# microsoft/tf-gnn-samples

Hardware: AMD Instinct MI355X
Metric: edges/sec (whole node), RGCN PPI h=256 training, distinct batches (the reference's epoch-loop definition) (higher is better)
Workload: dtype f32; 1 GPU; C2: RGCN on synthetic PPI-shaped batches (~16 graphs, ~1.88 M edges, ~32 k nodes each), 3 edge types [fwd,self,bkwd], h=256, 3 layers, sum aggregation, 1/in-de…; graphs_per_rank=64, max_nodes_in_batch=35964, input_pipeline=ResidentDataset, parallelism=dp1-by-graph

## Files before the change

tf_gnn_samples_amd/csrc/plan_resident.hip:

```cpp
#include "common.h"

using namespace relgnn;

namespace {

__device__ __forceinline__ int upper_slot(const int64_t* __restrict__ table, int n, int64_t x) {
  int lo = 0, hi = n;
  while (hi - lo > 1) {
    const int mid = (lo + hi) >> 1;
    if (table[mid] <= x) lo = mid; else hi = mid;
  }
  return lo;
}

struct BatchTables {
  const int64_t* ids;
  const int64_t* node_off_b;
  const int64_t* msg_off_b;
  const int64_t* edge_off_b;
  const int64_t* type_off_b;
  const int64_t* node_off_d;
  const int64_t* msg_off_d;
  const int64_t* edge_off_d;
  const int64_t* type_off_d;
  int32_t K, L;
  int64_t G;
};

__device__ __forceinline__ int32_t translate_message(const BatchTables& t, int32_t m_d, int l, int k, int64_t g) {
  const int64_t e = (int64_t)m_d - t.type_off_d[l] - t.edge_off_d[(int64_t)l * (t.G + 1) + g];
  return (int32_t)(t.type_off_b[l] + t.edge_off_b[(int64_t)l * (t.K + 1) + k] + e);
}

template <bool FULL>
__global__ __launch_bounds__(256) void assemble_by_target_kernel(
    BatchTables t, int64_t M, const int32_t* __restrict__ perm_d, const int32_t* __restrict__ col_d,
    int32_t* __restrict__ perm_b, int32_t* __restrict__ col_b, int32_t* __restrict__ inv_b,
    const float* __restrict__ w_t_d, int32_t* __restrict__ src_b, float* __restrict__ w_t_b) {
  __shared__ int first_slot;
  for (int64_t base = (int64_t)blockIdx.x * 1024; base < M; base += (int64_t)gridDim.x * 1024) {
    if (threadIdx.x == 0) first_slot = upper_slot(t.msg_off_b, t.K, base);
    __syncthreads();
    int k = first_slot;
    int64_t g = t.ids[k], slot_end = t.msg_off_b[k + 1];
    int64_t msg_delta = t.msg_off_d[g] - t.msg_off_b[k], node_delta = t.node_off_b[k] - t.node_off_d[g];
#pragma unroll
    for (int e = 0; e < 4; ++e) {
      const int64_t p = base + threadIdx.x + 256 * e;
      if (p >= M) break;
      if (p >= slot_end) {
        do { ++k; } while (p >= t.msg_off_b[k + 1]);
        g = t.ids[k]; slot_end = t.msg_off_b[k + 1];
        msg_delta = t.msg_off_d[g] - t.msg_off_b[k]; node_delta = t.node_off_b[k] - t.node_off_d[g];
      }
      const int64_t pd = p + msg_delta;
      const uint32_t c = (uint32_t)col_d[pd];
      const uint32_t cn = c / (uint32_t)t.L;
      const int64_t src = (int64_t)cn + node_delta;
      if (src_b) src_b[p] = (int32_t)src;
      if (w_t_b) w_t_b[p] = w_t_d[pd];
      if constexpr (FULL) {
        const int l = (int)(c - cn * (uint32_t)t.L);
        col_b[p] = (int32_t)(src * t.L + l);
        const int32_t mb = translate_message(t, perm_d[pd], l, k, g);
        perm_b[p] = mb;
        inv_b[mb] = (int32_t)p;
      }
    }
    __syncthreads();
  }
}

template <bool FULL>
__global__ __launch_bounds__(256) void assemble_by_source_kernel(
    BatchTables t, int64_t M, const int32_t* __restrict__ perm_d, const int32_t* __restrict__ frow_d,
    const int32_t* __restrict__ pos_d, int32_t* __restrict__ perm_b, int32_t* __restrict__ frow_b,
    int32_t* __restrict__ tgt_b, int32_t* __restrict__ pos_b, const float* __restrict__ w_s_d, float* __restrict__ w_s_b) {
  __shared__ int first_slot;
  for (int64_t base = (int64_t)blockIdx.x * 1024; base < M; base += (int64_t)gridDim.x * 1024) {
    if (threadIdx.x == 0) first_slot = upper_slot(t.msg_off_b, t.K, base);
    __syncthreads();
    int k = first_slot;
    int64_t g = t.ids[k], slot_end = t.msg_off_b[k + 1];
    int64_t msg_delta = t.msg_off_d[g] - t.msg_off_b[k], node_delta = t.node_off_b[k] - t.node_off_d[g];
#pragma unroll
    for (int e = 0; e < 4; ++e) {
      const int64_t q = base + threadIdx.x + 256 * e;
      if (q >= M) break;
      if (q >= slot_end) {
        do { ++k; } while (q >= t.msg_off_b[k + 1]);
        g = t.ids[k]; slot_end = t.msg_off_b[k + 1];
        msg_delta = t.msg_off_d[g] - t.msg_off_b[k]; node_delta = t.node_off_b[k] - t.node_off_d[g];
      }
      const int64_t qd = q + msg_delta;
      const uint32_t f = (uint32_t)frow_d[qd];
      const uint32_t fn = f / (uint32_t)t.L;
      const int64_t tgt = (int64_t)fn + node_delta;
      tgt_b[q] = (int32_t)tgt;
      if (w_s_b) w_s_b[q] = w_s_d[qd];
      if constexpr (FULL) {
        const int l = (int)(f - fn * (uint32_t)t.L);
        frow_b[q] = (int32_t)(tgt * t.L + l);
        perm_b[q] = translate_message(t, perm_d[qd], l, k, g);
        pos_b[q] = (int32_t)((int64_t)pos_d[qd] - msg_delta);
      }
    }
    __syncthreads();
  }
}

__global__ __launch_bounds__(256) void assemble_rowptr_kernel(
    BatchTables t, int64_t num_buckets, int64_t M, const int32_t* __restrict__ rowptr_t_d,
    const int32_t* __restrict__ rowptr_s_d, int32_t* __restrict__ rowptr_t_b, int32_t* __restrict__ rowptr_s_b) {
  for (int64_t b = blockIdx.x * (int64_t)blockDim.x + threadIdx.x; b <= num_buckets; b += (int64_t)gridDim.x * blockDim.x) {
    if (b == num_buckets) {
      rowptr_t_b[b] = (int32_t)M;
      rowptr_s_b[b] = (int32_t)M;
      continue;
    }
    const int64_t v = b / t.L;
    const int l = (int)(b - v * t.L);
    const int k = upper_slot(t.node_off_b, t.K, v);
    const int64_t g = t.ids[k];
    const int64_t bd = (v - t.node_off_b[k] + t.node_off_d[g]) * t.L + l;
    const int64_t shift = t.msg_off_b[k] - t.msg_off_d[g];
    rowptr_t_b[b] = (int32_t)((int64_t)rowptr_t_d[bd] + shift);
    rowptr_s_b[b] = (int32_t)((int64_t)rowptr_s_d[bd] + shift);
  }
}


__global__ __launch_bounds__(256) void gather_node_rows_kernel(BatchTables t, int64_t V, int32_t cols,
                                                               const uint32_t* __restrict__ src, uint32_t* __restrict__ dst) {
  __shared__ int first_slot;
  const int64_t total = V * cols;
  for (int64_t base = (int64_t)blockIdx.x * 1024; base < total; base += (int64_t)gridDim.x * 1024) {
    if (threadIdx.x == 0) {
      int lo = 0, hi = t.K;
      while (hi - lo > 1) {
        const int mid = (lo + hi) >> 1;
        if (t.node_off_b[mid] * cols <= base) lo = mid; else hi = mid;
      }
      first_slot = lo;
    }
    __syncthreads();
    int k = first_slot;
    int64_t slot_end = t.node_off_b[k + 1] * cols;
    int64_t delta = (t.node_off_d[t.ids[k]] - t.node_off_b[k]) * cols;
#pragma unroll
    for (int e = 0; e < 4; ++e) {
      const int64_t i = base + threadIdx.x + 256 * e;
      if (i < total) {
        if (i >= slot_end) {
          do { ++k; } while (i >= t.node_off_b[k + 1] * cols);
          slot_end = t.node_off_b[k + 1] * cols;
          delta = (t.node_off_d[t.ids[k]] - t.node_off_b[k]) * cols;
        }
        dst[i] = src[delta + i];
      }
    }
    __syncthreads();
  }
}

__global__ __launch_bounds__(256) void gather_degree_kernel(BatchTables t, int64_t V, int64_t N, const float* __restrict__ deg_d,
                                                            float* __restrict__ deg_b, int32_t* __restrict__ node_to_graph) {
  for (int64_t v = blockIdx.x * (int64_t)blockDim.x + threadIdx.x; v < V; v += (int64_t)gridDim.x * blockDim.x) {
    const int k = upper_slot(t.node_off_b, t.K, v);
    const int64_t vd = v - t.node_off_b[k] + t.node_off_d[t.ids[k]];
    for (int l = 0; l < t.L; ++l) deg_b[(int64_t)l * V + v] = deg_d[(int64_t)l * N + vd];
    node_to_graph[v] = k;
  }
}

__global__ __launch_bounds__(256) void gather_adjacency_kernel(BatchTables t, int64_t M, const int2* __restrict__ adj_d,
                                                               int2* __restrict__ adj_b) {
  for (int64_t p = blockIdx.x * (int64_t)blockDim.x + threadIdx.x; p < M; p += (int64_t)gridDim.x * blockDim.x) {
    const int l = upper_slot(t.type_off_b, t.L, p);
    const int64_t e = p - t.type_off_b[l];
    const int64_t* eob = t.edge_off_b + (int64_t)l * (t.K + 1);
    const int k = upper_slot(eob, t.K, e);
    const int64_t g = t.ids[k];
    const int64_t pd = t.type_off_d[l] + t.edge_off_d[(int64_t)l * (t.G + 1) + g] + (e - eob[k]);
    int2 a = adj_d[pd];
    const int off = (int)t.node_off_b[k];
    a.x += off; a.y += off;
    adj_b[p] = a;
  }
}

}

extern "C" {

int relgnn_batch_gather(const int64_t* ids, int32_t num_batch_graphs, int32_t num_edge_types, int64_t num_dataset_graphs,
                        const int64_t* node_off_b, const int64_t* edge_off_b, const int64_t* type_off_b,
                        const int64_t* node_off_d, const int64_t* edge_off_d, const int64_t* type_off_d, int64_t num_nodes,
                        int64_t num_messages, int64_t num_dataset_nodes, int32_t n_payloads, const void* const* h_payload_d,
                        const int32_t* h_payload_cols, void* const* h_payload_b, const float* deg_d, float* deg_b,
                        const int32_t* adj_d, int32_t* adj_b, int32_t* node_to_graph, void* stream) {
  if (num_batch_graphs < 0 || num_edge_types <= 0 || num_dataset_graphs < 0 || num_nodes < 0 || num_messages < 0 ||
      n_payloads < 0 || num_dataset_nodes < 0)
    return RELGNN_EINVAL;
  if (num_batch_graphs == 0 || num_nodes == 0) return RELGNN_OK;
  if (!ids || !node_off_b || !edge_off_b || !type_off_b || !node_off_d || !edge_off_d || !type_off_d) return RELGNN_EINVAL;
  if (n_payloads > 0 && (!h_payload_d || !h_payload_cols || !h_payload_b)) return RELGNN_EINVAL;
  hipStream_t st = as_stream(stream);
  BatchTables t{ids, node_off_b, nullptr, edge_off_b, type_off_b, node_off_d, nullptr, edge_off_d, type_off_d,
                num_batch_graphs, num_edge_types, num_dataset_graphs};
  for (int p = 0; p < n_payloads; ++p) {
    if (h_payload_cols[p] <= 0) continue;
    if (!h_payload_d[p] || !h_payload_b[p]) return RELGNN_EINVAL;
    gather_node_rows_kernel<<<flat_grid((num_nodes * h_payload_cols[p] + 3) / 4, 256), 256, 0, st>>>(
        t, num_nodes, h_payload_cols[p], (const uint32_t*)h_payload_d[p], (uint32_t*)h_payload_b[p]);
  }
  if (deg_b || node_to_graph) {
    if (!deg_d || !deg_b || !node_to_graph) return RELGNN_EINVAL;
    gather_degree_kernel<<<flat_grid(num_nodes, 256), 256, 0, st>>>(t, num_nodes, num_dataset_nodes, deg_d, deg_b, node_to_graph);
  }
  if (num_messages > 0 && adj_b) {
    if (!adj_d) return RELGNN_EINVAL;
    gather_adjacency_kernel<<<flat_grid(num_messages, 256), 256, 0, st>>>(t, num_messages, (const int2*)adj_d, (int2*)adj_b);
  }
  return launch_status();
}

int relgnn_plan_assemble(const int64_t* ids, int32_t num_batch_graphs, int32_t num_edge_types, int64_t num_dataset_graphs,
                         const int64_t* node_off_b, const int64_t* msg_off_b, const int64_t* edge_off_b,
                         const int64_t* type_off_b, const int64_t* node_off_d, const int64_t* msg_off_d,
                         const int64_t* edge_off_d, const int64_t* type_off_d, int64_t num_nodes, int64_t num_messages,
                         const int32_t* rowptr_t_d, const int32_t* perm_t_d, const int32_t* col_t_d,
                         const int32_t* rowptr_s_d, const int32_t* perm_s_d, const int32_t* frow_s_d,
                         const int32_t* pos_t_of_s_d, int32_t* rowptr_t, int32_t* perm_t, int32_t* col_t,
                         int32_t* inv_perm_t, int32_t* rowptr_s, int32_t* perm_s, int32_t* frow_s, int32_t* tgt_s,
                         int32_t* pos_t_of_s, const float* w_t_d, const float* w_s_d, int32_t* src_t, float* w_t, float* w_s,
                         void* stream) {
  if (num_batch_graphs < 0 || num_edge_types <= 0 || num_dataset_graphs < 0 || num_nodes < 0 || num_messages < 0)
    return RELGNN_EINVAL;
  const int64_t buckets = num_nodes * num_edge_types;
  if (buckets >= INT32_MAX || num_messages >= INT32_MAX) return RELGNN_EUNSUPPORTED;
  if (!rowptr_t || !rowptr_s) return RELGNN_EINVAL;
  hipStream_t st = as_stream(stream);
  if (num_batch_graphs == 0 || num_nodes == 0) {
    if (hipMemsetAsync(rowptr_t, 0, (size_t)(buckets + 1) * 4, st) != hipSuccess) return RELGNN_EHIP;
    if (hipMemsetAsync(rowptr_s, 0, (size_t)(buckets + 1) * 4, st) != hipSuccess) return RELGNN_EHIP;
    return RELGNN_OK;
  }
  if (!ids || !node_off_b || !msg_off_b || !edge_off_b || !type_off_b || !node_off_d || !msg_off_d || !edge_off_d ||
      !type_off_d || !rowptr_t_d || !rowptr_s_d)
    return RELGNN_EINVAL;
  BatchTables t{ids, node_off_b, msg_off_b, edge_off_b, type_off_b, node_off_d, msg_off_d, edge_off_d, type_off_d,
                num_batch_graphs, num_edge_types, num_dataset_graphs};
  assemble_rowptr_kernel<<<flat_grid(buckets + 1, 256), 256, 0, st>>>(t, buckets, num_messages, rowptr_t_d, rowptr_s_d,
                                                                      rowptr_t, rowptr_s);
  if (num_messages > 0) {
    const bool full = perm_t || col_t || inv_perm_t || perm_s || frow_s || pos_t_of_s;
    if (full && (!perm_t || !col_t || !inv_perm_t || !perm_s || !frow_s || !pos_t_of_s || !perm_t_d || !perm_s_d || !pos_t_of_s_d))
      return RELGNN_EINVAL;
    if (!col_t_d || !frow_s_d || !tgt_s) return RELGNN_EINVAL;
    if (!full && !src_t) return RELGNN_EINVAL;
    if ((w_t && !w_t_d) || (w_s && !w_s_d)) return RELGNN_EINVAL;
    const dim3 grid = flat_grid((num_messages + 3) / 4, 256);
    if (full) {
      assemble_by_target_kernel<true><<<grid, 256, 0, st>>>(t, num_messages, perm_t_d, col_t_d, perm_t, col_t, inv_perm_t,
                                                            w_t_d, src_t, w_t);
      assemble_by_source_kernel<true><<<grid, 256, 0, st>>>(t, num_messages, perm_s_d, frow_s_d, pos_t_of_s_d, perm_s, frow_s,
                                                            tgt_s, pos_t_of_s, w_s_d, w_s);
    } else {
      assemble_by_target_kernel<false><<<grid, 256, 0, st>>>(t, num_messages, nullptr, col_t_d, nullptr, nullptr, nullptr,
                                                             w_t_d, src_t, w_t);
      assemble_by_source_kernel<false><<<grid, 256, 0, st>>>(t, num_messages, nullptr, frow_s_d, nullptr, nullptr, nullptr,
                                                             tgt_s, nullptr, w_s_d, w_s);
    }
  }
  return launch_status();
}

}
```

tf_gnn_samples_amd/csrc/train_utils.hip:

```cpp
#include "common.h"
#include "adam_element.h"
#include "norm_tree.h"
#include "../../include/relgnn_subgraph_norm.h"
#include <type_traits>

using namespace relgnn;

namespace {

struct MtArgs {
  float* p[RELGNN_MT_MAX];
  const float* g[RELGNN_MT_MAX];
  float* m[RELGNN_MT_MAX];
  float* v[RELGNN_MT_MAX];
  long long n[RELGNN_MT_MAX];
};

struct NormArgs {
  const float* g[RELGNN_MT_MAX];
  long long n[RELGNN_MT_MAX];
};

__device__ __forceinline__ double block_sum_1024(double x, double* red) {
#pragma unroll
  for (int off = 32; off >= 1; off >>= 1) x += __shfl_xor(x, off);
  const int wave = threadIdx.x >> 6, lane = threadIdx.x & 63;
  if (lane == 0) red[wave] = x;
  __syncthreads();
  double t = 0.0;
  if (threadIdx.x == 0)
    for (int i = 0; i < (int)(blockDim.x >> 6); ++i) t += red[i];
  __syncthreads();
  return t;
}

__global__ __launch_bounds__(kNormBlock) void mt_l2norm_partial_kernel(NormArgs a, double* __restrict__ partial) {
  __shared__ double red[4];
  const int t = blockIdx.y;
  const float* g = a.g[t];
  const long long n = a.n[t];
  double acc = 0.0;
  for (long long i = (long long)blockIdx.x * blockDim.x + threadIdx.x; i < n; i += (long long)gridDim.x * blockDim.x) {
    const double x = g[i];
    acc += x * x;
  }
  const double sum = norm_block_partial(acc, red);
  if (threadIdx.x == 0) partial[(long long)t * kNormChunks + blockIdx.x] = sum;
}

__global__ __launch_bounds__(64) void mt_l2norm_final_kernel(const double* __restrict__ partial, float* __restrict__ norms) {
  const int t = blockIdx.x;
  const float norm = norm_of_partials(partial + (long long)t * kNormChunks);
  if (threadIdx.x == 0) norms[t] = norm;
}

__global__ void adam_step_size_kernel(float* __restrict__ state, float lr, float b1, float b2) {
  const float t = state[0] + 1.f;
  state[0] = t;
  state[1] = lr * sqrtf(1.f - powf(b2, t)) / (1.f - powf(b1, t));
}

__global__ __launch_bounds__(256) void mt_adam_clip_kernel(MtArgs a, const float* __restrict__ norms, float clip,
                                                           float lr_t, const float* __restrict__ d_lr_t, float b1, float b2,
                                                           float eps) {
  if (d_lr_t) lr_t = d_lr_t[0];
  const int t = blockIdx.y;
  const long long n = a.n[t];
  const long long chunk = 4096;
  const long long beg = (long long)blockIdx.x * chunk;
  if (beg >= n) return;
  const long long end = min(n, beg + chunk);
  float scale = 1.f;
  if (clip > 0.f) {
    const float nrm = norms[t];
    scale = clip / fmaxf(nrm, clip);
  }
  float* p = a.p[t];
  const float* g = a.g[t];
  float* m = a.m[t];
  float* v = a.v[t];
  for (long long i = beg + threadIdx.x; i < end; i += blockDim.x) {
    float pi = p[i], mi = m[i], vi = v[i];
    adam_element(pi, g[i] * scale, mi, vi, lr_t, b1, b2, eps);
    m[i] = mi;
    v[i] = vi;
    p[i] = pi;
  }
}

struct SgdArgs {
  float* p[RELGNN_MT_MAX];
  const float* g[RELGNN_MT_MAX];
  long long n[RELGNN_MT_MAX];
};

__device__ __forceinline__ void rmsprop_element(float& p, float g, float& ms, float& mom, float scale, float lr,
                                                float one_minus_decay, float momentum, float eps) {
#pragma clang fp contract(off)
  const float gi = g * scale;
  const float d = gi * gi - ms;
  ms = ms + d * one_minus_decay;
  const float num = lr * gi;
  mom = mom * momentum + num / sqrtf(ms + eps);
  p = p - mom;
}

__device__ __forceinline__ void sgd_element(float& p, float g, float scale, float lr) {
#pragma clang fp contract(off)
  const float gi = g * scale;
  p = p - lr * gi;
}

__device__ __forceinline__ float clip_scale(const float* __restrict__ norms, int t, float clip) {
  return clip > 0.f ? clip / fmaxf(norms[t], clip) : 1.f;
}

__device__ __forceinline__ bool aligned16(const void* a, const void* b, const void* c = nullptr, const void* d = nullptr) {
  return ((reinterpret_cast<uintptr_t>(a) | reinterpret_cast<uintptr_t>(b) | reinterpret_cast<uintptr_t>(c) |
           reinterpret_cast<uintptr_t>(d)) & 15) == 0;
}

__global__ __launch_bounds__(256) void mt_rmsprop_clip_kernel(MtArgs a, const float* __restrict__ norms, float clip, float lr,
                                                              float decay, float momentum, float eps) {
  const int t = blockIdx.y;
  const long long n = a.n[t];
  const long long beg = (long long)blockIdx.x * 4096;
  if (beg >= n) return;
  const int len = (int)min(n - beg, 4096LL);
  const float scale = clip_scale(norms, t, clip);
  const float omd = 1.f - decay;
  float* p = a.p[t] + beg;
  const float* g = a.g[t] + beg;
  float* ms = a.m[t] + beg;
  float* mom = a.v[t] + beg;
  const int n4 = aligned16(p, g, ms, mom) ? len / 4 : 0;
  for (int i = threadIdx.x; i < n4; i += blockDim.x) {
    float4 pv = reinterpret_cast<float4*>(p)[i], sv = reinterpret_cast<float4*>(ms)[i], mv = reinterpret_cast<float4*>(mom)[i];
    const float4 gv = reinterpret_cast<const float4*>(g)[i];
    rmsprop_element(pv.x, gv.x, sv.x, mv.x, scale, lr, omd, momentum, eps);
    rmsprop_element(pv.y, gv.y, sv.y, mv.y, scale, lr, omd, momentum, eps);
    rmsprop_element(pv.z, gv.z, sv.z, mv.z, scale, lr, omd, momentum, eps);
    rmsprop_element(pv.w, gv.w, sv.w, mv.w, scale, lr, omd, momentum, eps);
    reinterpret_cast<float4*>(ms)[i] = sv;
    reinterpret_cast<float4*>(mom)[i] = mv;
    reinterpret_cast<float4*>(p)[i] = pv;
  }
  for (int i = 4 * n4 + threadIdx.x; i < len; i += blockDim.x) {
    float pi = p[i], si = ms[i], mi = mom[i];
    rmsprop_element(pi, g[i], si, mi, scale, lr, omd, momentum, eps);
    ms[i] = si;
    mom[i] = mi;
    p[i] = pi;
  }
}

__global__ __launch_bounds__(256) void mt_sgd_clip_kernel(SgdArgs a, const float* __restrict__ norms, float clip, float lr) {
  const int t = blockIdx.y;
  const long long n = a.n[t];
  const long long beg = (long long)blockIdx.x * 4096;
  if (beg >= n) return;
  const int len = (int)min(n - beg, 4096LL);
  const float scale = clip_scale(norms, t, clip);
  float* p = a.p[t] + beg;
  const float* g = a.g[t] + beg;
  const int n4 = aligned16(p, g) ? len / 4 : 0;
  for (int i = threadIdx.x; i < n4; i += blockDim.x) {
    float4 pv = reinterpret_cast<float4*>(p)[i];
    const float4 gv = reinterpret_cast<const float4*>(g)[i];
    sgd_element(pv.x, gv.x, scale, lr);
    sgd_element(pv.y, gv.y, scale, lr);
    sgd_element(pv.z, gv.z, scale, lr);
    sgd_element(pv.w, gv.w, scale, lr);
    reinterpret_cast<float4*>(p)[i] = pv;
  }
  for (int i = 4 * n4 + threadIdx.x; i < len; i += blockDim.x) {
    float pi = p[i];
    sgd_element(pi, g[i], scale, lr);
    p[i] = pi;
  }
}

struct CeAcc {
  double loss;
  int tp, fp, fn;
};

__device__ __forceinline__ void ce_element(float x, float z, CeAcc& a) {
  const float e = expf(-fabsf(x));
  a.loss += (double)(fmaxf(x, 0.f) - x * z + log1pf(e));
  const bool pred = sigmoid_label(x, e);
  const int zi = (int)z;
  a.tp += (pred && zi != 0) ? 1 : 0;
  a.fp += (pred && zi != 1) ? 1 : 0;
  a.fn += (!pred && zi != 0) ? 1 : 0;
}

__global__ __launch_bounds__(1024) void sigmoid_ce_stats_kernel(const float* __restrict__ logits,
                                                                const float* __restrict__ labels, long long n,
                                                                double* __restrict__ partial) {
  __shared__ double red[16];
  CeAcc a = {0.0, 0, 0, 0};
  const long long tid = (long long)blockIdx.x * blockDim.x + threadIdx.x, nth = (long long)gridDim.x * blockDim.x;
  const bool vec = ((reinterpret_cast<uintptr_t>(logits) | reinterpret_cast<uintptr_t>(labels)) & 15) == 0;
  const long long n4 = vec ? n / 4 : 0;
  const float4* x4 = reinterpret_cast<const float4*>(logits);
  const float4* z4 = reinterpret_cast<const float4*>(labels);
  for (long long i = tid; i < n4; i += nth) {
    const float4 x = x4[i], z = z4[i];
    ce_element(x.x, z.x, a); ce_element(x.y, z.y, a); ce_element(x.z, z.z, a); ce_element(x.w, z.w, a);
  }
  for (long long i = 4 * n4 + tid; i < n; i += nth) ce_element(logits[i], labels[i], a);
  double s;
  s = block_sum_1024(a.loss, red);       if (threadIdx.x == 0) partial[blockIdx.x * 4 + 0] = s;
  s = block_sum_1024((double)a.tp, red); if (threadIdx.x == 0) partial[blockIdx.x * 4 + 1] = s;
  s = block_sum_1024((double)a.fp, red); if (threadIdx.x == 0) partial[blockIdx.x * 4 + 2] = s;
  s = block_sum_1024((double)a.fn, red); if (threadIdx.x == 0) partial[blockIdx.x * 4 + 3] = s;
}

__global__ __launch_bounds__(256) void sigmoid_ce_stats_final_kernel(const double* __restrict__ partial, int nblk,
                                                                     float mean_scale, float* __restrict__ stats) {
  __shared__ double red[4][4];
  __shared__ double tot[4];
  const int b = threadIdx.x;
  double v[4];
#pragma unroll
  for (int k = 0; k < 4; ++k) v[k] = b < nblk ? partial[b * 4 + k] : 0.0;
#pragma unroll
  for (int k = 0; k < 4; ++k) {
#pragma unroll
    for (int off = 32; off >= 1; off >>= 1) v[k] += __shfl_xor(v[k], off);
  }
  const int wave = b >> 6, lane = b & 63;
  if (lane == 0) {
#pragma unroll
    for (int k = 0; k < 4; ++k) red[wave][k] = v[k];
  }
  __syncthreads();
  if (b < 4) {
    const double s = (red[0][b] + red[1][b]) + (red[2][b] + red[3][b]);
    stats[b] = (float)s;
    tot[b] = s;
  }
  __syncthreads();
  if (b == 0) {
    const double precision = tot[1] / (tot[1] + tot[2]);
    const double recall = tot[1] / (tot[1] + tot[3]);
    stats[4] = (float)((2.0 * precision * recall) / (precision + recall));
    stats[5] = (float)tot[0] * mean_scale;
  }
}

__global__ __launch_bounds__(256) void sigmoid_ce_bwd_kernel(const float* __restrict__ logits,
                                                             const float* __restrict__ labels, long long n,
                                                             const float* __restrict__ g_mean, float mean_scale,
                                                             const float* __restrict__ g_total, float* __restrict__ gl) {
  float gs = 0.f;
  if (g_mean) gs = g_mean[0] * mean_scale;
  if (g_total) gs = g_mean ? gs + g_total[0] : g_total[0];
  for (long long i = (long long)blockIdx.x * blockDim.x + threadIdx.x; i < n; i += (long long)gridDim.x * blockDim.x) {
    const float x = logits[i];
    gl[i] = gs * (1.f / (1.f + expf(-x)) - labels[i]);
  }
}

__global__ __launch_bounds__(256) void sigmoid_ce_bwd_padded_kernel(const float* __restrict__ logits,
                                                                    const float* __restrict__ labels, long long rows, int cols,
                                                                    int ldg, const float* __restrict__ g_mean, float mean_scale,
                                                                    const float* __restrict__ g_total, float* __restrict__ gl) {
  float gs = 0.f;
  if (g_mean) gs = g_mean[0] * mean_scale;
  if (g_total) gs = g_mean ? gs + g_total[0] : g_total[0];
  const long long n = rows * ldg;
// ... 149 lines not shown
                                                                      const int* __restrict__ labels, const float* __restrict__ mask,
                                                                      const float* __restrict__ weights, float denominator,
                                                                      long long rows, int cols, const float* __restrict__ g_loss,
                                                                      const float* __restrict__ g_total, float* __restrict__ gl,
                                                                      long long ldg) {
  constexpr int kRowsPerBlock = 256 / W;
  const int j = threadIdx.x % W, g = threadIdx.x / W;
  float gs = 0.f;
  if (g_loss) gs = g_loss[0] / denominator;
  if (g_total) gs = g_loss ? gs + g_total[0] : g_total[0];
  for (long long base = (long long)blockIdx.x * kRowsPerBlock; base < rows; base += (long long)gridDim.x * kRowsPerBlock) {
    const long long r = base + g;
    const bool valid = r < rows;
    const float* row = logits + (valid ? r : 0) * ld;
    const RowLse a = row_lse<W>(row, valid ? cols : 0, j);
    if (!valid) continue;
    const float mk = mask[r];
    const int label = labels[r];
    const float scale = (mk * weights[r]) * gs, inv = 1.f / (1.f + a.t);
    float* out = gl + r * ldg;
    for (int c = j; c < (int)ldg; c += W) {
      float v = 0.f;
      if (c < cols && mk != 0.f) v = scale * (expf(row[c] - a.m) * inv - (c == label ? 1.f : 0.f));
      out[c] = v;
    }
  }
}

constexpr int kSoftmaxBlocks = 256;

static inline int softmax_grid(long long rows, int w) {
  const long long per_block = 256 / w;
  long long g = (rows + per_block - 1) / per_block;
  return (int)(g < 1 ? 1 : (g > kSoftmaxBlocks ? kSoftmaxBlocks : g));
}

template <bool kWeighted>
int softmax_ce_stats_launch(const float* logits, int64_t ld, const int32_t* labels, const float* mask, const float* weights,
                            float denominator, int64_t rows, int32_t cols, float* stats, void* workspace, size_t workspace_bytes,
                            void* stream) {
  if (rows < 0 || cols < 1 || ld < cols || !stats || (kWeighted && (denominator == 0.f || denominator != denominator)))
    return RELGNN_EINVAL;
  if (!workspace || workspace_bytes < (size_t)kSoftmaxBlocks * (kWeighted ? 4 : 3) * sizeof(double)) return RELGNN_ENOSPC;
  if (rows > 0 && (!logits || !labels || !mask || (kWeighted && !weights))) return RELGNN_EINVAL;
  hipStream_t st = as_stream(stream);
  double* partial = static_cast<double*>(workspace);
  int nblk = 0;
  if (rows > 0) {
    const int w = softmax_group_width(cols);
    nblk = softmax_grid(rows, w);
    auto walk = [&](auto width) {
      constexpr int W = decltype(width)::value;
      if constexpr (kWeighted) softmax_ce_weighted_stats_kernel<W><<<nblk, 256, 0, st>>>(logits, ld, labels, mask, weights, rows, cols, partial);
      else softmax_ce_stats_kernel<W><<<nblk, 256, 0, st>>>(logits, ld, labels, mask, rows, cols, partial);
    };
    if (w == 1) walk(std::integral_constant<int, 1>{});
    else if (w == 16) walk(std::integral_constant<int, 16>{});
    else walk(std::integral_constant<int, 64>{});
  }
  if constexpr (kWeighted) softmax_ce_weighted_stats_final_kernel<<<1, 256, 0, st>>>(partial, nblk, denominator, stats);
  else softmax_ce_stats_final_kernel<<<1, 256, 0, st>>>(partial, nblk, stats);
  return launch_status();
}

template <bool kWeighted>
int softmax_ce_bwd_launch(const float* logits, int64_t ld, const int32_t* labels, const float* mask, const float* weights,
                          float denominator, int64_t rows, int32_t cols, const float* stats, const float* g_loss,
                          const float* g_total, float* glogits, int64_t ldg, void* stream) {
  if (rows < 0 || cols < 1 || ld < cols || ldg < cols || ldg > INT32_MAX
      || (kWeighted && (denominator == 0.f || denominator != denominator)))
    return RELGNN_EINVAL;
  if (rows == 0) return RELGNN_OK;
  if (!logits || !labels || !mask || (kWeighted ? !weights : !stats) || (!g_loss && !g_total) || !glogits) return RELGNN_EINVAL;
  hipStream_t st = as_stream(stream);
  const int w = softmax_group_width(cols);
  const int64_t per_block = 256 / w;
  const unsigned nblk = flat_grid((rows + per_block - 1) / per_block * 256, 256);
  auto walk = [&](auto width) {
    constexpr int W = decltype(width)::value;
    if constexpr (kWeighted)
      softmax_ce_weighted_bwd_kernel<W><<<nblk, 256, 0, st>>>(logits, ld, labels, mask, weights, denominator, rows, cols, g_loss, g_total, glogits, ldg);
    else
      softmax_ce_bwd_kernel<W><<<nblk, 256, 0, st>>>(logits, ld, labels, mask, rows, cols, stats, g_loss, g_total, glogits, ldg);
  };
  if (w == 1) walk(std::integral_constant<int, 1>{});
  else if (w == 16) walk(std::integral_constant<int, 16>{});
  else walk(std::integral_constant<int, 64>{});
  return launch_status();
}

constexpr int kStatsBlocks = 256;

}

extern "C" {

size_t relgnn_mt_l2norm_workspace_bytes(void) { return (size_t)RELGNN_MT_MAX * kNormChunks * sizeof(double); }

int relgnn_mt_l2norm(const float* const* h_grads, const int64_t* h_sizes, int32_t n, float* norms, void* workspace,
                     size_t workspace_bytes, void* stream) {
  if (n < 0 || n > RELGNN_MT_MAX) return RELGNN_EINVAL;
  if (n == 0) return RELGNN_OK;
  if (!h_grads || !h_sizes || !norms) return RELGNN_EINVAL;
  if (!workspace || workspace_bytes < relgnn_mt_l2norm_workspace_bytes()) return RELGNN_ENOSPC;
  NormArgs a;
  for (int i = 0; i < n; ++i) {
    if (h_sizes[i] < 0 || (h_sizes[i] > 0 && !h_grads[i])) return RELGNN_EINVAL;
    a.g[i] = h_grads[i];
    a.n[i] = h_sizes[i];
  }
  double* partial = static_cast<double*>(workspace);
  mt_l2norm_partial_kernel<<<dim3(kNormChunks, (unsigned)n), kNormBlock, 0, as_stream(stream)>>>(a, partial);
  mt_l2norm_final_kernel<<<n, 64, 0, as_stream(stream)>>>(partial, norms);
  return launch_status();
}

int relgnn_adam_step_size(float* d_state, float lr, float beta1, float beta2, void* stream) {
  if (!d_state) return RELGNN_EINVAL;
  adam_step_size_kernel<<<1, 1, 0, as_stream(stream)>>>(d_state, lr, beta1, beta2);
  return launch_status();
}

static int mt_adam_clip_impl(float* const* h_params, const float* const* h_grads, float* const* h_m, float* const* h_v,
                             const int64_t* h_sizes, int32_t n, const float* norms, float clip, float lr_t,
                             const float* d_lr_t, float beta1, float beta2, float eps, void* stream);

int relgnn_mt_adam_clip(float* const* h_params, const float* const* h_grads, float* const* h_m, float* const* h_v,
                        const int64_t* h_sizes, int32_t n, const float* norms, float clip, float lr_t, float beta1,
                        float beta2, float eps, void* stream) {
  return mt_adam_clip_impl(h_params, h_grads, h_m, h_v, h_sizes, n, norms, clip, lr_t, nullptr, beta1, beta2, eps, stream);
}

int relgnn_mt_adam_clip_devlr(float* const* h_params, const float* const* h_grads, float* const* h_m, float* const* h_v,
                              const int64_t* h_sizes, int32_t n, const float* norms, float clip, const float* d_lr_t,
                              float beta1, float beta2, float eps, void* stream) {
  if (!d_lr_t) return RELGNN_EINVAL;
  return mt_adam_clip_impl(h_params, h_grads, h_m, h_v, h_sizes, n, norms, clip, 0.f, d_lr_t, beta1, beta2, eps, stream);
}

static int mt_adam_clip_impl(float* const* h_params, const float* const* h_grads, float* const* h_m, float* const* h_v,
                             const int64_t* h_sizes, int32_t n, const float* norms, float clip, float lr_t,
                             const float* d_lr_t, float beta1, float beta2, float eps, void* stream) {
  if (n < 0 || n > RELGNN_MT_MAX) return RELGNN_EINVAL;
  if (n == 0) return RELGNN_OK;
  if (!h_params || !h_grads || !h_m || !h_v || !h_sizes || (clip > 0.f && !norms)) return RELGNN_EINVAL;
  MtArgs a;
  long long maxn = 0;
  for (int i = 0; i < n; ++i) {
    if (h_sizes[i] < 0) return RELGNN_EINVAL;
    a.p[i] = h_params[i]; a.g[i] = h_grads[i]; a.m[i] = h_m[i]; a.v[i] = h_v[i]; a.n[i] = h_sizes[i];
    if (h_sizes[i] > maxn) maxn = h_sizes[i];
  }
  if (maxn == 0) return RELGNN_OK;
  dim3 grid((unsigned)((maxn + 4095) / 4096), (unsigned)n);
  mt_adam_clip_kernel<<<grid, 256, 0, as_stream(stream)>>>(a, norms, clip, lr_t, d_lr_t, beta1, beta2, eps);
  return launch_status();
}

int relgnn_mt_rmsprop_clip(float* const* h_params, const float* const* h_grads, float* const* h_ms, float* const* h_mom,
                           const int64_t* h_sizes, int32_t n, const float* norms, float clip, float lr, float decay,
                           float momentum, float eps, void* stream) {
  if (n < 0 || n > RELGNN_MT_MAX) return RELGNN_EINVAL;
  if (n == 0) return RELGNN_OK;
  if (!h_params || !h_grads || !h_ms || !h_mom || !h_sizes || (clip > 0.f && !norms)) return RELGNN_EINVAL;
  MtArgs a;
  long long maxn = 0;
  for (int i = 0; i < n; ++i) {
    if (h_sizes[i] < 0 || (h_sizes[i] > 0 && (!h_params[i] || !h_grads[i] || !h_ms[i] || !h_mom[i]))) return RELGNN_EINVAL;
    a.p[i] = h_params[i]; a.g[i] = h_grads[i]; a.m[i] = h_ms[i]; a.v[i] = h_mom[i]; a.n[i] = h_sizes[i];
    if (h_sizes[i] > maxn) maxn = h_sizes[i];
  }
  if (maxn == 0) return RELGNN_OK;
  dim3 grid((unsigned)((maxn + 4095) / 4096), (unsigned)n);
  mt_rmsprop_clip_kernel<<<grid, 256, 0, as_stream(stream)>>>(a, norms, clip, lr, decay, momentum, eps);
  return launch_status();
}

int relgnn_mt_sgd_clip(float* const* h_params, const float* const* h_grads, const int64_t* h_sizes, int32_t n,
                       const float* norms, float clip, float lr, void* stream) {
  if (n < 0 || n > RELGNN_MT_MAX) return RELGNN_EINVAL;
  if (n == 0) return RELGNN_OK;
  if (!h_params || !h_grads || !h_sizes || (clip > 0.f && !norms)) return RELGNN_EINVAL;
  SgdArgs a;
  long long maxn = 0;
  for (int i = 0; i < n; ++i) {
    if (h_sizes[i] < 0 || (h_sizes[i] > 0 && (!h_params[i] || !h_grads[i]))) return RELGNN_EINVAL;
    a.p[i] = h_params[i]; a.g[i] = h_grads[i]; a.n[i] = h_sizes[i];
    if (h_sizes[i] > maxn) maxn = h_sizes[i];
  }
  if (maxn == 0) return RELGNN_OK;
  dim3 grid((unsigned)((maxn + 4095) / 4096), (unsigned)n);
  mt_sgd_clip_kernel<<<grid, 256, 0, as_stream(stream)>>>(a, norms, clip, lr);
  return launch_status();
}

size_t relgnn_sigmoid_ce_stats_workspace_bytes(void) { return (size_t)kStatsBlocks * 4 * sizeof(double); }

int relgnn_sigmoid_ce_stats(const float* logits, const float* labels, int64_t n, float mean_scale, float* stats,
                            void* workspace, size_t workspace_bytes, void* stream) {
  if (n < 0 || !stats) return RELGNN_EINVAL;
  if (!workspace || workspace_bytes < relgnn_sigmoid_ce_stats_workspace_bytes()) return RELGNN_ENOSPC;
  if (n > 0 && (!logits || !labels)) return RELGNN_EINVAL;
  hipStream_t st = as_stream(stream);
  int nblk = (int)((n + 1023) / 1024);
  if (nblk < 1) nblk = 1;
  if (nblk > kStatsBlocks) nblk = kStatsBlocks;
  sigmoid_ce_stats_kernel<<<nblk, 1024, 0, st>>>(logits, labels, n, static_cast<double*>(workspace));
  sigmoid_ce_stats_final_kernel<<<1, 256, 0, st>>>(static_cast<const double*>(workspace), nblk, mean_scale, stats);
  return launch_status();
}

int relgnn_sigmoid_ce_bwd(const float* logits, const float* labels, int64_t n, const float* g_mean, float mean_scale,
                          const float* g_total, float* glogits, void* stream) {
  if (n < 0) return RELGNN_EINVAL;
  if (n == 0) return RELGNN_OK;
  if (!logits || !labels || (!g_mean && !g_total) || !glogits) return RELGNN_EINVAL;
  sigmoid_ce_bwd_kernel<<<flat_grid(n, 256), 256, 0, as_stream(stream)>>>(logits, labels, n, g_mean, mean_scale, g_total,
                                                                          glogits);
  return launch_status();
}

int relgnn_sigmoid_ce_bwd_padded(const float* logits, const float* labels, int64_t rows, int32_t cols, const float* g_mean,
                                 float mean_scale, const float* g_total, float* glogits, int32_t ldg, void* stream) {
  if (rows < 0 || cols < 0 || ldg < cols) return RELGNN_EINVAL;
  if (rows == 0 || ldg == 0) return RELGNN_OK;
  if (!logits || !labels || (!g_mean && !g_total) || !glogits) return RELGNN_EINVAL;
  sigmoid_ce_bwd_padded_kernel<<<flat_grid(rows * ldg, 256), 256, 0, as_stream(stream)>>>(logits, labels, rows, cols, ldg, g_mean,
                                                                                          mean_scale, g_total, glogits);
  return launch_status();
}

size_t relgnn_softmax_ce_stats_workspace_bytes(void) { return (size_t)kSoftmaxBlocks * 3 * sizeof(double); }

int relgnn_softmax_ce_stats(const float* logits, int64_t ld, const int32_t* labels, const float* mask, int64_t rows, int32_t cols,
                            float* stats, void* workspace, size_t workspace_bytes, void* stream) {
  return softmax_ce_stats_launch<false>(logits, ld, labels, mask, nullptr, 0.f, rows, cols, stats, workspace, workspace_bytes, stream);
}

int relgnn_softmax_ce_bwd(const float* logits, int64_t ld, const int32_t* labels, const float* mask, int64_t rows, int32_t cols,
                          const float* stats, const float* g_loss, const float* g_total, float* glogits, int64_t ldg,
                          void* stream) {
  return softmax_ce_bwd_launch<false>(logits, ld, labels, mask, nullptr, 0.f, rows, cols, stats, g_loss, g_total, glogits, ldg, stream);
}

size_t relgnn_softmax_ce_weighted_stats_workspace_bytes(void) { return (size_t)kSoftmaxBlocks * 4 * sizeof(double); }

int relgnn_softmax_ce_weighted_stats(const float* logits, int64_t ld, const int32_t* labels, const float* mask, const float* weights,
                                     float denominator, int64_t rows, int32_t cols, float* stats, void* workspace,
                                     size_t workspace_bytes, void* stream) {
  return softmax_ce_stats_launch<true>(logits, ld, labels, mask, weights, denominator, rows, cols, stats, workspace, workspace_bytes,
                                       stream);
}

int relgnn_softmax_ce_weighted_bwd(const float* logits, int64_t ld, const int32_t* labels, const float* mask, const float* weights,
                                   float denominator, int64_t rows, int32_t cols, const float* g_loss, const float* g_total,
                                   float* glogits, int64_t ldg, void* stream) {
  return softmax_ce_bwd_launch<true>(logits, ld, labels, mask, weights, denominator, rows, cols, nullptr, g_loss, g_total, glogits, ldg,
                                     stream);
}

}
```

Baseline: 1.086 billion edges/sec.

## Fuse batch gather and plan assembly kernels into role-dispatched launches; vectorize Adam

```diff
diff --git a/tf_gnn_samples_amd/csrc/plan_resident.hip b/tf_gnn_samples_amd/csrc/plan_resident.hip
--- a/tf_gnn_samples_amd/csrc/plan_resident.hip
+++ b/tf_gnn_samples_amd/csrc/plan_resident.hip
@@ -33,12 +33,12 @@
 }
 
 template <bool FULL>
-__global__ __launch_bounds__(256) void assemble_by_target_kernel(
-    BatchTables t, int64_t M, const int32_t* __restrict__ perm_d, const int32_t* __restrict__ col_d,
-    int32_t* __restrict__ perm_b, int32_t* __restrict__ col_b, int32_t* __restrict__ inv_b,
+__device__ __forceinline__ void assemble_by_target(
+    unsigned block, unsigned blocks, const BatchTables& t, int64_t M, const int32_t* __restrict__ perm_d,
+    const int32_t* __restrict__ col_d, int32_t* __restrict__ perm_b, int32_t* __restrict__ col_b, int32_t* __restrict__ inv_b,
     const float* __restrict__ w_t_d, int32_t* __restrict__ src_b, float* __restrict__ w_t_b) {
   __shared__ int first_slot;
-  for (int64_t base = (int64_t)blockIdx.x * 1024; base < M; base += (int64_t)gridDim.x * 1024) {
+  for (int64_t base = (int64_t)block * 1024; base < M; base += (int64_t)blocks * 1024) {
     if (threadIdx.x == 0) first_slot = upper_slot(t.msg_off_b, t.K, base);
     __syncthreads();
     int k = first_slot;
@@ -72,12 +72,13 @@
 }
 
 template <bool FULL>
-__global__ __launch_bounds__(256) void assemble_by_source_kernel(
-    BatchTables t, int64_t M, const int32_t* __restrict__ perm_d, const int32_t* __restrict__ frow_d,
-    const int32_t* __restrict__ pos_d, int32_t* __restrict__ perm_b, int32_t* __restrict__ frow_b,
-    int32_t* __restrict__ tgt_b, int32_t* __restrict__ pos_b, const float* __restrict__ w_s_d, float* __restrict__ w_s_b) {
+__device__ __forceinline__ void assemble_by_source(
+    unsigned block, unsigned blocks, const BatchTables& t, int64_t M, const int32_t* __restrict__ perm_d,
+    const int32_t* __restrict__ frow_d, const int32_t* __restrict__ pos_d, int32_t* __restrict__ perm_b,
+    int32_t* __restrict__ frow_b, int32_t* __restrict__ tgt_b, int32_t* __restrict__ pos_b, const float* __restrict__ w_s_d,
+    float* __restrict__ w_s_b) {
   __shared__ int first_slot;
-  for (int64_t base = (int64_t)blockIdx.x * 1024; base < M; base += (int64_t)gridDim.x * 1024) {
+  for (int64_t base = (int64_t)block * 1024; base < M; base += (int64_t)blocks * 1024) {
     if (threadIdx.x == 0) first_slot = upper_slot(t.msg_off_b, t.K, base);
     __syncthreads();
     int k = first_slot;
@@ -109,10 +110,10 @@
   }
 }
 
-__global__ __launch_bounds__(256) void assemble_rowptr_kernel(
-    BatchTables t, int64_t num_buckets, int64_t M, const int32_t* __restrict__ rowptr_t_d,
+__device__ __forceinline__ void assemble_rowptr(
+    unsigned block, unsigned blocks, const BatchTables& t, int64_t num_buckets, int64_t M, const int32_t* __restrict__ rowptr_t_d,
     const int32_t* __restrict__ rowptr_s_d, int32_t* __restrict__ rowptr_t_b, int32_t* __restrict__ rowptr_s_b) {
-  for (int64_t b = blockIdx.x * (int64_t)blockDim.x + threadIdx.x; b <= num_buckets; b += (int64_t)gridDim.x * blockDim.x) {
+  for (int64_t b = block * (int64_t)blockDim.x + threadIdx.x; b <= num_buckets; b += (int64_t)blocks * blockDim.x) {
     if (b == num_buckets) {
       rowptr_t_b[b] = (int32_t)M;
       rowptr_s_b[b] = (int32_t)M;
@@ -130,11 +131,11 @@
 }
 
 
-__global__ __launch_bounds__(256) void gather_node_rows_kernel(BatchTables t, int64_t V, int32_t cols,
-                                                               const uint32_t* __restrict__ src, uint32_t* __restrict__ dst) {
+__device__ __forceinline__ void gather_node_rows(unsigned block, unsigned blocks, const BatchTables& t, int64_t V, int32_t cols,
+                                                 const uint32_t* __restrict__ src, uint32_t* __restrict__ dst) {
   __shared__ int first_slot;
   const int64_t total = V * cols;
-  for (int64_t base = (int64_t)blockIdx.x * 1024; base < total; base += (int64_t)gridDim.x * 1024) {
+  for (int64_t base = (int64_t)block * 1024; base < total; base += (int64_t)blocks * 1024) {
     if (threadIdx.x == 0) {
       int lo = 0, hi = t.K;
       while (hi - lo > 1) {
@@ -163,9 +164,10 @@
   }
 }
 
-__global__ __launch_bounds__(256) void gather_degree_kernel(BatchTables t, int64_t V, int64_t N, const float* __restrict__ deg_d,
-                                                            float* __restrict__ deg_b, int32_t* __restrict__ node_to_graph) {
-  for (int64_t v = blockIdx.x * (int64_t)blockDim.x + threadIdx.x; v < V; v += (int64_t)gridDim.x * blockDim.x) {
+__device__ __forceinline__ void gather_degree(unsigned block, unsigned blocks, const BatchTables& t, int64_t V, int64_t N,
+                                              const float* __restrict__ deg_d, float* __restrict__ deg_b,
+                                              int32_t* __restrict__ node_to_graph) {
+  for (int64_t v = block * (int64_t)blockDim.x + threadIdx.x; v < V; v += (int64_t)blocks * blockDim.x) {
     const int k = upper_slot(t.node_off_b, t.K, v);
     const int64_t vd = v - t.node_off_b[k] + t.node_off_d[t.ids[k]];
     for (int l = 0; l < t.L; ++l) deg_b[(int64_t)l * V + v] = deg_d[(int64_t)l * N + vd];
@@ -173,9 +175,9 @@
   }
 }
 
-__global__ __launch_bounds__(256) void gather_adjacency_kernel(BatchTables t, int64_t M, const int2* __restrict__ adj_d,
-                                                               int2* __restrict__ adj_b) {
-  for (int64_t p = blockIdx.x * (int64_t)blockDim.x + threadIdx.x; p < M; p += (int64_t)gridDim.x * blockDim.x) {
+__device__ __forceinline__ void gather_adjacency(unsigned block, unsigned blocks, const BatchTables& t, int64_t M,
+                                                 const int2* __restrict__ adj_d, int2* __restrict__ adj_b) {
+  for (int64_t p = block * (int64_t)blockDim.x + threadIdx.x; p < M; p += (int64_t)blocks * blockDim.x) {
     const int l = upper_slot(t.type_off_b, t.L, p);
     const int64_t e = p - t.type_off_b[l];
     const int64_t* eob = t.edge_off_b + (int64_t)l * (t.K + 1);
@@ -187,6 +189,63 @@
     a.x += off; a.y += off;
     adj_b[p] = a;
   }
+}
+
+template <int R>
+struct RoleEnds {
+  unsigned end[R];
+  unsigned push(int r, unsigned blocks) { return end[r] = (r ? end[r - 1] : 0u) + blocks; }
+};
+
+template <int R>
+__device__ __forceinline__ int find_role(const RoleEnds<R>& e, unsigned& block, unsigned& blocks) {
+  int role = 0;
+  unsigned first = 0;
+#pragma unroll
+  for (int i = 0; i + 1 < R; ++i)
+    if (blockIdx.x >= e.end[i]) { role = i + 1; first = e.end[i]; }
+  block = blockIdx.x - first;
+  blocks = e.end[role] - first;
+  return role;
+}
+
+constexpr int kFusedPayloads = 8;
+struct GatherPayloads {
+  const uint32_t* src[kFusedPayloads];
+  uint32_t* dst[kFusedPayloads];
+  int32_t cols[kFusedPayloads];
+};
+
+__global__ __launch_bounds__(256) void batch_gather_kernel(BatchTables t, RoleEnds<kFusedPayloads + 2> ends, GatherPayloads pl,
+                                                           int64_t V, int64_t M, int64_t N, const float* __restrict__ deg_d,
+                                                           float* __restrict__ deg_b, int32_t* __restrict__ node_to_graph,
+                                                           const int2* __restrict__ adj_d, int2* __restrict__ adj_b) {
+  unsigned block, blocks;
+  const int role = find_role(ends, block, blocks);
+  if (role < kFusedPayloads) gather_node_rows(block, blocks, t, V, pl.cols[role], pl.src[role], pl.dst[role]);
+  else if (role == kFusedPayloads) gather_degree(block, blocks, t, V, N, deg_d, deg_b, node_to_graph);
+  else gather_adjacency(block, blocks, t, M, adj_d, adj_b);
+}
+
+__global__ __launch_bounds__(256) void gather_node_rows_kernel(BatchTables t, int64_t V, int32_t cols,
+                                                               const uint32_t* __restrict__ src, uint32_t* __restrict__ dst) {
+  gather_node_rows(blockIdx.x, gridDim.x, t, V, cols, src, dst);
+}
+
+template <bool FULL>
+__global__ __launch_bounds__(256) void plan_assemble_kernel(
+    BatchTables t, RoleEnds<3> ends, int64_t num_buckets, int64_t M, const int32_t* __restrict__ rowptr_t_d,
+    const int32_t* __restrict__ perm_t_d, const int32_t* __restrict__ col_t_d, const int32_t* __restrict__ rowptr_s_d,
+    const int32_t* __restrict__ perm_s_d, const int32_t* __restrict__ frow_s_d, const int32_t* __restrict__ pos_t_of_s_d,
+    int32_t* __restrict__ rowptr_t, int32_t* __restrict__ perm_t, int32_t* __restrict__ col_t, int32_t* __restrict__ inv_perm_t,
+    int32_t* __restrict__ rowptr_s, int32_t* __restrict__ perm_s, int32_t* __restrict__ frow_s, int32_t* __restrict__ tgt_s,
+    int32_t* __restrict__ pos_t_of_s, const float* __restrict__ w_t_d, const float* __restrict__ w_s_d,
+    int32_t* __restrict__ src_t, float* __restrict__ w_t, float* __restrict__ w_s) {
+  unsigned block, blocks;
+  const int role = find_role(ends, block, blocks);
+  if (role == 0) assemble_by_target<FULL>(block, blocks, t, M, perm_t_d, col_t_d, perm_t, col_t, inv_perm_t, w_t_d, src_t, w_t);
+  else if (role == 1) assemble_by_source<FULL>(block, blocks, t, M, perm_s_d, frow_s_d, pos_t_of_s_d, perm_s, frow_s, tgt_s, pos_t_of_s, w_s_d, w_s);
+  else assemble_rowptr(block, blocks, t, num_buckets, M, rowptr_t_d, rowptr_s_d, rowptr_t, rowptr_s);
 }
 
 }
@@ -205,23 +264,41 @@
   if (num_batch_graphs == 0 || num_nodes == 0) return RELGNN_OK;
   if (!ids || !node_off_b || !edge_off_b || !type_off_b || !node_off_d || !edge_off_d || !type_off_d) return RELGNN_EINVAL;
   if (n_payloads > 0 && (!h_payload_d || !h_payload_cols || !h_payload_b)) return RELGNN_EINVAL;
+  for (int p = 0; p < n_payloads; ++p)
+    if (h_payload_cols[p] > 0 && (!h_payload_d[p] || !h_payload_b[p])) return RELGNN_EINVAL;
+  const bool node_tables = deg_b || node_to_graph;
+  if (node_tables && (!deg_d || !deg_b || !node_to_graph)) return RELGNN_EINVAL;
+  const bool adjacency = num_messages > 0 && adj_b;
+  if (adjacency && !adj_d) return RELGNN_EINVAL;
   hipStream_t st = as_stream(stream);
   BatchTables t{ids, node_off_b, nullptr, edge_off_b, type_off_b, node_off_d, nullptr, edge_off_d, type_off_d,
                 num_batch_graphs, num_edge_types, num_dataset_graphs};
+  RoleEnds<kFusedPayloads + 2> ends;
+  GatherPayloads pl;
+  unsigned grid = 0;
+  int fused = 0;
   for (int p = 0; p < n_payloads; ++p) {
     if (h_payload_cols[p] <= 0) continue;
-    if (!h_payload_d[p] || !h_payload_b[p]) return RELGNN_EINVAL;
-    gather_node_rows_kernel<<<flat_grid((num_nodes * h_payload_cols[p] + 3) / 4, 256), 256, 0, st>>>(
-        t, num_nodes, h_payload_cols[p], (const uint32_t*)h_payload_d[p], (uint32_t*)h_payload_b[p]);
-  }
-  if (deg_b || node_to_graph) {
-    if (!deg_d || !deg_b || !node_to_graph) return RELGNN_EINVAL;
-    gather_degree_kernel<<<flat_grid(num_nodes, 256), 256, 0, st>>>(t, num_nodes, num_dataset_nodes, deg_d, deg_b, node_to_graph);
-  }
-  if (num_messages > 0 && adj_b) {
-    if (!adj_d) return RELGNN_EINVAL;
-    gather_adjacency_kernel<<<flat_grid(num_messages, 256), 256, 0, st>>>(t, num_messages, (const int2*)adj_d, (int2*)adj_b);
-  }
+    const unsigned blocks = flat_grid((num_nodes * h_payload_cols[p] + 3) / 4, 256);
+    if (fused < kFusedPayloads) {
+      pl.src[fused] = (const uint32_t*)h_payload_d[p];
+      pl.dst[fused] = (uint32_t*)h_payload_b[p];
+      pl.cols[fused] = h_payload_cols[p];
+      grid = ends.push(fused++, blocks);
+    } else {
+      gather_node_rows_kernel<<<blocks, 256, 0, st>>>(t, num_nodes, h_payload_cols[p], (const uint32_t*)h_payload_d[p],
+                                                      (uint32_t*)h_payload_b[p]);
+    }
+  }
+  for (int r = fused; r < kFusedPayloads; ++r) {
+    pl.src[r] = nullptr; pl.dst[r] = nullptr; pl.cols[r] = 0;
+    grid = ends.push(r, 0);
+  }
+  grid = ends.push(kFusedPayloads, node_tables ? flat_grid(num_nodes, 256) : 0u);
+  grid = ends.push(kFusedPayloads + 1, adjacency ? flat_grid(num_messages, 256) : 0u);
+  if (grid > 0)
+    batch_gather_kernel<<<grid, 256, 0, st>>>(t, ends, pl, num_nodes, num_messages, num_dataset_nodes, deg_d, deg_b, node_to_graph,
+                                              (const int2*)adj_d, (int2*)adj_b);
   return launch_status();
 }
 
@@ -249,30 +326,30 @@
   if (!ids || !node_off_b || !msg_off_b || !edge_off_b || !type_off_b || !node_off_d || !msg_off_d || !edge_off_d ||
       !type_off_d || !rowptr_t_d || !rowptr_s_d)
     return RELGNN_EINVAL;
-  BatchTables t{ids, node_off_b, msg_off_b, edge_off_b, type_off_b, node_off_d, msg_off_d, edge_off_d, type_off_d,
-                num_batch_graphs, num_edge_types, num_dataset_graphs};
-  assemble_rowptr_kernel<<<flat_grid(buckets + 1, 256), 256, 0, st>>>(t, buckets, num_messages, rowptr_t_d, rowptr_s_d,
-                                                                      rowptr_t, rowptr_s);
+  bool full = false;
   if (num_messages > 0) {
-    const bool full = perm_t || col_t || inv_perm_t || perm_s || frow_s || pos_t_of_s;
+    full = perm_t || col_t || inv_perm_t || perm_s || frow_s || pos_t_of_s;
     if (full && (!perm_t || !col_t || !inv_perm_t || !perm_s || !frow_s || !pos_t_of_s || !perm_t_d || !perm_s_d || !pos_t_of_s_d))
       return RELGNN_EINVAL;
     if (!col_t_d || !frow_s_d || !tgt_s) return RELGNN_EINVAL;
     if (!full && !src_t) return RELGNN_EINVAL;
     if ((w_t && !w_t_d) || (w_s && !w_s_d)) return RELGNN_EINVAL;
-    const dim3 grid = flat_grid((num_messages + 3) / 4, 256);
-    if (full) {
-      assemble_by_target_kernel<true><<<grid, 256, 0, st>>>(t, num_messages, perm_t_d, col_t_d, perm_t, col_t, inv_perm_t,
-                                                            w_t_d, src_t, w_t);
-      assemble_by_source_kernel<true><<<grid, 256, 0, st>>>(t, num_messages, perm_s_d, frow_s_d, pos_t_of_s_d, perm_s, frow_s,
-                                                            tgt_s, pos_t_of_s, w_s_d, w_s);
-    } else {
-      assemble_by_target_kernel<false><<<grid, 256, 0, st>>>(t, num_messages, nullptr, col_t_d, nullptr, nullptr, nullptr,
-                                                             w_t_d, src_t, w_t);
-      assemble_by_source_kernel<false><<<grid, 256, 0, st>>>(t, num_messages, nullptr, frow_s_d, nullptr, nullptr, nullptr,
-                                                             tgt_s, nullptr, w_s_d, w_s);
-    }
-  }
+  }
+  BatchTables t{ids, node_off_b, msg_off_b, edge_off_b, type_off_b, node_off_d, msg_off_d, edge_off_d, type_off_d,
+                num_batch_graphs, num_edge_types, num_dataset_graphs};
+  const unsigned per_message = num_messages > 0 ? flat_grid((num_messages + 3) / 4, 256) : 0u;
+  RoleEnds<3> ends;
+  ends.push(0, per_message);
+  ends.push(1, per_message);
+  const unsigned grid = ends.push(2, flat_grid(buckets + 1, 256));
+  if (full)
+    plan_assemble_kernel<true><<<grid, 256, 0, st>>>(t, ends, buckets, num_messages, rowptr_t_d, perm_t_d, col_t_d, rowptr_s_d,
+                                                     perm_s_d, frow_s_d, pos_t_of_s_d, rowptr_t, perm_t, col_t, inv_perm_t, rowptr_s,
+                                                     perm_s, frow_s, tgt_s, pos_t_of_s, w_t_d, w_s_d, src_t, w_t, w_s);
+  else
+    plan_assemble_kernel<false><<<grid, 256, 0, st>>>(t, ends, buckets, num_messages, rowptr_t_d, nullptr, col_t_d, rowptr_s_d,
+                                                      nullptr, frow_s_d, nullptr, rowptr_t, nullptr, nullptr, nullptr, rowptr_s,
+                                                      nullptr, nullptr, tgt_s, nullptr, w_t_d, w_s_d, src_t, w_t, w_s);
   return launch_status();
 }
 
diff --git a/tf_gnn_samples_amd/csrc/train_utils.hip b/tf_gnn_samples_amd/csrc/train_utils.hip
--- a/tf_gnn_samples_amd/csrc/train_utils.hip
+++ b/tf_gnn_samples_amd/csrc/train_utils.hip
@@ -60,26 +60,44 @@
   state[1] = lr * sqrtf(1.f - powf(b2, t)) / (1.f - powf(b1, t));
 }
 
+__device__ __forceinline__ bool aligned16(const void* a, const void* b, const void* c = nullptr, const void* d = nullptr) {
+  return ((reinterpret_cast<uintptr_t>(a) | reinterpret_cast<uintptr_t>(b) | reinterpret_cast<uintptr_t>(c) |
+           reinterpret_cast<uintptr_t>(d)) & 15) == 0;
+}
+
+constexpr int kAdamChunk = 1024;
+
 __global__ __launch_bounds__(256) void mt_adam_clip_kernel(MtArgs a, const float* __restrict__ norms, float clip,
                                                            float lr_t, const float* __restrict__ d_lr_t, float b1, float b2,
                                                            float eps) {
   if (d_lr_t) lr_t = d_lr_t[0];
   const int t = blockIdx.y;
   const long long n = a.n[t];
-  const long long chunk = 4096;
-  const long long beg = (long long)blockIdx.x * chunk;
+  const long long beg = (long long)blockIdx.x * kAdamChunk;
   if (beg >= n) return;
-  const long long end = min(n, beg + chunk);
+  const int len = (int)min(n - beg, (long long)kAdamChunk);
   float scale = 1.f;
   if (clip > 0.f) {
     const float nrm = norms[t];
     scale = clip / fmaxf(nrm, clip);
   }
-  float* p = a.p[t];
-  const float* g = a.g[t];
-  float* m = a.m[t];
-  float* v = a.v[t];
-  for (long long i = beg + threadIdx.x; i < end; i += blockDim.x) {
+  float* p = a.p[t] + beg;
+  const float* g = a.g[t] + beg;
+  float* m = a.m[t] + beg;
+  float* v = a.v[t] + beg;
+  const int n4 = aligned16(p, g, m, v) ? len / 4 : 0;
+  for (int i = threadIdx.x; i < n4; i += blockDim.x) {
+    float4 pv = reinterpret_cast<float4*>(p)[i], mv = reinterpret_cast<float4*>(m)[i], vv = reinterpret_cast<float4*>(v)[i];
+    const float4 gv = reinterpret_cast<const float4*>(g)[i];
+    adam_element(pv.x, gv.x * scale, mv.x, vv.x, lr_t, b1, b2, eps);
+    adam_element(pv.y, gv.y * scale, mv.y, vv.y, lr_t, b1, b2, eps);
+    adam_element(pv.z, gv.z * scale, mv.z, vv.z, lr_t, b1, b2, eps);
+    adam_element(pv.w, gv.w * scale, mv.w, vv.w, lr_t, b1, b2, eps);
+    reinterpret_cast<float4*>(m)[i] = mv;
+    reinterpret_cast<float4*>(v)[i] = vv;
+    reinterpret_cast<float4*>(p)[i] = pv;
+  }
+  for (int i = 4 * n4 + threadIdx.x; i < len; i += blockDim.x) {
     float pi = p[i], mi = m[i], vi = v[i];
     adam_element(pi, g[i] * scale, mi, vi, lr_t, b1, b2, eps);
     m[i] = mi;
@@ -113,11 +131,6 @@
 
 __device__ __forceinline__ float clip_scale(const float* __restrict__ norms, int t, float clip) {
   return clip > 0.f ? clip / fmaxf(norms[t], clip) : 1.f;
-}
-
-__device__ __forceinline__ bool aligned16(const void* a, const void* b, const void* c = nullptr, const void* d = nullptr) {
-  return ((reinterpret_cast<uintptr_t>(a) | reinterpret_cast<uintptr_t>(b) | reinterpret_cast<uintptr_t>(c) |
-           reinterpret_cast<uintptr_t>(d)) & 15) == 0;
 }
 
 __global__ __launch_bounds__(256) void mt_rmsprop_clip_kernel(MtArgs a, const float* __restrict__ norms, float clip, float lr,
@@ -573,7 +586,7 @@
     if (h_sizes[i] > maxn) maxn = h_sizes[i];
   }
   if (maxn == 0) return RELGNN_OK;
-  dim3 grid((unsigned)((maxn + 4095) / 4096), (unsigned)n);
+  dim3 grid((unsigned)((maxn + kAdamChunk - 1) / kAdamChunk), (unsigned)n);
   mt_adam_clip_kernel<<<grid, 256, 0, as_stream(stream)>>>(a, norms, clip, lr_t, d_lr_t, beta1, beta2, eps);
   return launch_status();
 }
```

New measurement: 1.098 billion edges/sec, median of 6. 1.01x the previous value.
